# Keshav-Madhav/3d-spatial-sim-for-boid-and-nbody

Hardware: AMD Instinct MI355X
Metric: body-steps/sec (N-body Barnes-Hut, theta=0.5) (higher is better)
Workload: dtype f64 pair forces for the waves of 64 bodies whose densest quarter has G*rho*dt^2 > tau - and for every wave while most of the system qualifies (entered above a third of the waves, left below a quarter; library default 'auto') -, f32 pair forces with f64 sums for the others; f64 opening-test ties, f64; 1 GPU; galaxy_1m_bh; distribution=galaxy, bodies_per_gpu=1000000, bodies_total=1000000, method=barnes_hut, force_precision=auto, parallelism=single GPU

## Files before the change

### 3d-spatial-sim-for-boid-and-nbody_amd/csrc/common.h

```cpp
#pragma once
#include <hip/hip_runtime.h>
#include <stdint.h>
#include <stdio.h>
#include <string>

namespace nbmi {

void set_error(const char *fmt, ...);
const char *get_error();
void clear_error();

#define NBMI_HIP_CHECK(expr)                                                                \
    do {                                                                                    \
        hipError_t _e = (expr);                                                             \
        if (_e != hipSuccess) {                                                             \
            (void)hipGetLastError();  \
            nbmi::set_error("%s failed: %s (%s:%d)", #expr, hipGetErrorString(_e), __FILE__, \
                            __LINE__);                                                      \
            return -2;                                                                      \
        }                                                                                   \
    } while (0)

struct Moment {
    double m, ml, x, xl, y, yl, z, zl;
};

struct RadixConfig {
    int digit_bits = 0, threads = 0;
};
struct RadixHist;
bool radix_config_ok(RadixConfig cfg);
size_t radix_temp_bytes_u64(size_t n, int bits);
size_t radix_temp_bytes_u32(size_t n, int bits);
hipError_t radix_sort_pairs_u64(void *temp, size_t temp_bytes, const uint64_t *kin, uint64_t *kout, const uint32_t *vin,
                                uint32_t *vout, size_t n, int begin_bit, int end_bit, hipStream_t s, RadixConfig cfg = {});
hipError_t radix_sort_pairs_u32(void *temp, size_t temp_bytes, const uint32_t *kin, uint32_t *kout, const uint32_t *vin,
                                uint32_t *vout, size_t n, int begin_bit, int end_bit, hipStream_t s, RadixConfig cfg = {});
size_t radix_keys_temp_bytes_u64(size_t n, int bits);
size_t radix_keys_temp_bytes_u32(size_t n, int bits);
hipError_t radix_sort_keys_u64(void *temp, size_t temp_bytes, const uint64_t *kin, uint64_t *kout, size_t n, int begin_bit,
                               int end_bit, hipStream_t s, RadixConfig cfg = {}, bool have_hist = false);
hipError_t radix_sort_keys_u32(void *temp, size_t temp_bytes, const uint32_t *kin, uint32_t *kout, size_t n, int begin_bit,
                               int end_bit, hipStream_t s, RadixConfig cfg = {});
hipError_t radix_keys_prepare_u64(void *temp, size_t temp_bytes, size_t n, int begin_bit, int end_bit, RadixConfig cfg,
                                  hipStream_t s, RadixHist *out);
hipError_t radix_init_temp(void *temp, hipStream_t s);
hipError_t radix_error_word(const void *temp, unsigned *out, hipStream_t s);
const void *radix_error_device_word(const void *temp);

}
struct nbmi_sim;
// ... 42 lines not shown
```

### 3d-spatial-sim-for-boid-and-nbody_amd/csrc/nbmi.hip

```cpp
#include <math.h>
#include <stdarg.h>
#include <stddef.h>
#include <stdlib.h>
#include <string.h>

#include <algorithm>
#include <type_traits>
#include <utility>
#include <vector>

#include "../../include/nbmi.h"
#include "common.h"
#include "radix_hist.h"
#include "hilbert.h"
#include "visible.h"

namespace nbmi {
static thread_local char g_err[512] = "";
void set_error(const char *fmt, ...) {
    va_list ap;
    va_start(ap, fmt);
    vsnprintf(g_err, sizeof(g_err), fmt, ap);
    va_end(ap);
}
// ... 538 lines not shown
                                              double &M, double &mx, double &my, double &mz) {
    const double4 s0 = S[r], s1 = S[e];
    M = s1.x - s0.x; mx = s1.y - s0.y; my = s1.z - s0.z; mz = s1.w - s0.w;
    const int64_t ur = r >> kSubShift, ue = e >> kSubShift;
    if (ue != ur) {
        const Moment a = T[ur], b = T[ue];
        M += dd_diff(dd{b.m, b.ml}, dd{a.m, a.ml});
        mx += dd_diff(dd{b.x, b.xl}, dd{a.x, a.xl});
        my += dd_diff(dd{b.y, b.yl}, dd{a.y, a.yl});
        mz += dd_diff(dd{b.z, b.zl}, dd{a.z, a.zl});
    }
}

__device__ __forceinline__ void write_sentinel(Node *__restrict__ nodes, int32_t *__restrict__ node_ref, int64_t total,
                                               int64_t link_base = 0) {
    Node sn;
    sn.cx = sn.cy = sn.cz = 1.0e30f;
    sn.gm = 0.f; sn.s2t = 0.f;
    sn.next_off = (unsigned)(total + link_base) * kNodeBytes;
    nodes[total] = sn;
    if (node_ref) node_ref[total] = -1;
}

template <int TILE>
__global__ __launch_bounds__(kBlock) void k_emit_tile(const int32_t *__restrict__ delta, const int32_t *__restrict__ PexL,
                                                      const int32_t *__restrict__ subPex, const double4 *__restrict__ S,
                                                      const Moment *__restrict__ T, const float4 *__restrict__ posm_s,
                                                      const uint64_t *__restrict__ hi_s,
                                                      const uint64_t *__restrict__ lo_s, int64_t n, int64_t capacity,
                                                      double eps, double inv_theta2, Node *__restrict__ nodes,
                                                      Node64 *__restrict__ nodes64, uint8_t *__restrict__ node_level,
                                                      int32_t *__restrict__ node_ref, double4 *__restrict__ diag64,
                                                      NodeD *__restrict__ nodesd , Bodies cur,
                                                      const uint32_t *__restrict__ perm, double G, TreeInfo *info, int hilbert,
                                                      int64_t link_base ) {
    __shared__ uint8_t tree[2 * TILE];
    __shared__ uint8_t dprev;
    __shared__ uint32_t cells[(2 * TILE)];
    const int t = threadIdx.x;
    const int64_t base = (int64_t)blockIdx.x * TILE;
    const int64_t total = n + pex_at(PexL, subPex, n);
    if (blockIdx.x == 0 && t == 0) {
        info->num_nodes = total;
        info->walk_nodes = total;
        info->band2 = 2u * band_half_ulps(__longlong_as_double((long long)info->maxabs_bits), eps);
        if (total + 1 > capacity) {
            info->error = 1;
            if (info->sticky_error == 0) {
                info->sticky_error = 1;
                info->sticky_nodes = total;
            }
        } else {
            write_sentinel(nodes, node_ref, total, link_base);
            if (nodesd) nodesd[total] = NodeD{1.0e30, 1.0e30, 1.0e30, 0.0, 0.0f, (unsigned)(total + link_base) * kNodeDBytes};
        }
    }
    if (total + 1 > capacity) return;
    for (int i = t; i < TILE; i += kBlock) {
        const int64_t r = base + i;
        tree[TILE + i] = (uint8_t)((r < n ? delta[r] : -1) + 1);
    }
// ... 8 lines not shown
    }
    const int64_t q_tile = pex_at(PexL, subPex, base < n ? base : n);
    const int64_t tile_end = base + TILE < n ? base + TILE : n;
    const int64_t ncell = pex_at(PexL, subPex, tile_end) - q_tile;
    const int64_t nnode = (tile_end - base) + ncell;
    const int64_t idx0 = base + q_tile;
    const double bounds = info->bounds;
    const unsigned bandk = band_half_ulps(__longlong_as_double((long long)info->maxabs_bits), eps);
    for (int64_t c0 = 0; c0 < nnode; c0 += (2 * TILE)) {
        for (int i = t; i < TILE; i += kBlock) {
            const int64_t r = base + i;
            if (r >= n) break;
            const int d = (int)tree[TILE + i] - 1;
            const int dp = (int)(i > 0 ? tree[TILE + i - 1] : dprev) - 1;
            const int cnt = d > dp ? d - dp : 0;
            const int64_t s0 = i + (pex_at(PexL, subPex, r) - q_tile) - c0;
            for (int k = 0; k <= cnt; k++) {
                const int64_t c = s0 + k;
                if (c >= 0 && c < (2 * TILE)) cells[c] = ((uint32_t)i << 6) | (uint32_t)k;
            }
        }
        __syncthreads();
        const int64_t here = nnode - c0 < (2 * TILE) ? nnode - c0 : (2 * TILE);
        for (int64_t c = t; c < here; c += kBlock) {
            const uint32_t cl = cells[c];
            const int i = (int)(cl >> 6), k = (int)(cl & 63u);
            const int64_t r = base + i;
            const int64_t idx = idx0 + c0 + c;
            const int d = (int)tree[TILE + i] - 1;
            const int dp = (int)(i > 0 ? tree[TILE + i - 1] : dprev) - 1;
            const int cnt = d > dp ? d - dp : 0;
            if (k == cnt) {
                const float4 p = posm_s[r];
                Node lf;
                lf.cx = p.x; lf.cy = p.y; lf.cz = p.z; lf.gm = p.w;
                lf.s2t = 0.0f;
                lf.next_off = (unsigned)(idx + 1 + link_base) * kNodeBytes;
                nodes[idx] = lf;
                if (diag64) {
                    const uint32_t j = perm[r];
                    diag64[idx] = make_double4(cur.x[j], cur.y[j], cur.z[j], G * cur.m[j]);
                }
                if (nodesd) {
                    const uint32_t j = perm[r];
                    nodesd[idx] = NodeD{cur.x[j], cur.y[j], cur.z[j], G * cur.m[j], 0.0f, (unsigned)(idx + 1 + link_base) * kNodeDBytes};
                }
                if (node_ref) {
                    node_ref[idx] = (int32_t)r;
                    node_level[idx] = (uint8_t)((d > dp ? d : dp) + 1);
                }
                continue;
            }
            const int lev = dp + 1 + k;
            unsigned h = (unsigned)(TILE + i);
            bool found = false;
            for (;;) {
                if ((int)tree[h] <= lev) { found = true; break; }
                while ((h & 1u) && h > 1u) h >>= 1;
                if (h == 1u) break;
                h += 1u;
            }
            int64_t e;
            if (found) {
                while (h < (unsigned)TILE) {
                    h <<= 1;
                    if ((int)tree[h] > lev) h += 1u;
                }
                e = base + (int64_t)(h - (unsigned)TILE) + 1;
            } else {
                const uint64_t kh = hi_s[r];
                const bool deep = lev > 21;
                const uint64_t kl = lo_s ? lo_s[r] : (deep ? low_word_of(nullptr, cur, perm[r], hilbert, info) : 0ull);
                auto reaches = [&](int64_t u) {
                    const uint64_t hu = hi_s[u];
// ... 5 lines not shown
                    const int64_t u = ok + step;
                    if (u >= n) { bad = n; break; }
                    if (reaches(u)) { ok = u; step <<= 1; }
                    else { bad = u; break; }
                }
                while (bad - ok > 1) {
                    const int64_t mid = ok + ((bad - ok) >> 1);
                    if (reaches(mid)) ok = mid; else bad = mid;
                }
                e = bad;
            }
            double M, mx, my, mz;
            range_moments(S, T, r, e, M, mx, my, mz);
            double cx = 0.0, cy = 0.0, cz = 0.0;
            if (M > 0.0) { cx = mx / M; cy = my / M; cz = mz / M; }
            const double size = ldexp(bounds, 1 - lev);
            Node nd;
            nd.cx = (float)cx; nd.cy = (float)cy; nd.cz = (float)cz;
            nd.gm = (float)M;
            const float s2t = (float)(size * size * inv_theta2);
            nd.s2t = __int_as_float(__float_as_int(s2t) + (int)bandk);
            const int64_t nxt = e + pex_at(PexL, subPex, e) + link_base;
            nd.next_off = (unsigned)nxt * kNodeBytes;
            nodes[idx] = nd;
            if (nodesd) nodesd[idx] = NodeD{cx, cy, cz, M, __int_as_float(__float_as_int(s2t) + (int)kBand64), (unsigned)nxt * kNodeDBytes};
            nodes64[idx] = Node64{cx, cy, cz, ldexp(bounds, -lev)};
            if (diag64) diag64[idx] = make_double4(cx, cy, cz, M);
            if (node_ref) {
                node_ref[idx] = (int32_t)r;
                node_level[idx] = (uint8_t)lev;
            }
        }
        __syncthreads();
    }
}

__global__ __launch_bounds__(kBlock) void k_max_level(const int32_t *__restrict__ delta, int64_t n, TreeInfo *info) {
    __shared__ int red[kBlock / 64];
    int m = -1;
    for (int64_t i = (int64_t)blockIdx.x * kBlock + threadIdx.x; i < n; i += (int64_t)gridDim.x * kBlock) {
        const int d = delta[i];
        m = d > m ? d : m;
    }
#pragma unroll
    for (int o = 32; o > 0; o >>= 1) {
        const int other = __shfl_xor(m, o);
        m = other > m ? other : m;
    }
    if ((threadIdx.x & 63) == 0) red[threadIdx.x >> 6] = m;
    __syncthreads();
    if (threadIdx.x == 0) {
        for (int w = 1; w < kBlock / 64; w++) m = red[w] > m ? red[w] : m;
        atomicMax(&info->max_level, m + 1);
    }
// ... 2801 lines not shown
        int kind = 0;
        int64_t steps = 0, seq = 0;
    } frame_slot[NBMI_FRAME_SLOTS];
    hipStream_t frame_stream = nullptr;
    int64_t frame_seq = 0;
    uint8_t *vis_flag = nullptr;
    uint32_t *vis_slot = nullptr, *vis_tiles = nullptr;
    int xcd_chunk = 0;
    int xcd_balance = 1;
    int *xcd_bounds = nullptr;
    unsigned *wave_cycles = nullptr;
    unsigned char *wave_flag = nullptr;
    int32_t *sub_flag = nullptr;
    double step_dt = 0.0;
    double uniform_gm = -1.0;
    double max_gm = 0.0;
    int owner_all64 = -1;
    double owner_dt = 0.0;
    int balance_blocks = 0;
    hipStream_t side = nullptr;
    hipEvent_t ev_walked = nullptr, ev_cut = nullptr;
    bool cut_pending = false;
    int walk_block = kBlock;
    bool keys_lean = true;
    bool lean_build = false;
    bool sort_packed = true;
    uint64_t *packed = nullptr, *packed_s = nullptr;
    nbmi::RadixConfig sort_cfg;
    int sort_fused_hist = -1;
    int sort_bits = 0;
    bool maxabs_fused = false;
    bool fuse_maxabs = true;
    bool hilbert = true;
    double *diag_phi = nullptr;
    int32_t *diag_cnt = nullptr;
    double *diag_part = nullptr;
    long long *diag_partc = nullptr;
    double4 *diag_pot = nullptr;
    TreeInfo *side_info = nullptr;
    double *knn_r2 = nullptr, *knn_mass = nullptr;
    double4 *knn_rows = nullptr;
    unsigned long long *knn_evals = nullptr;
    int32_t *fof_parent = nullptr, *fof_root = nullptr, *fof_minid = nullptr, *fof_cnt = nullptr;
    uint32_t *fof_wleaf = nullptr;
    unsigned long long *fof_counters = nullptr;
    bool fof_ready = false, fof_cat_ready = false;
// ... 213 lines not shown
    with_bool(lean, [&](auto l) {
        k_gather_scan<decltype(l)::value><<<(int)((n_live + 1 + kScanTile - 1) / kScanTile), kBlock, 0, st>>>(
            cur, s->perm, s->hi_s, key_lo, n_live, s->G, s->posm_s, s->p64_s, lean ? nullptr : s->lo_s, s->delta, s->S, s->Pex,
            s->sub_tot, s->sub_cnt, auto_prec(s) ? s->wave_flag : nullptr, s->sub_flag,
            auto_prec(s) ? (float)(s->prec_tau / (s->step_dt * s->step_dt)) : 0.f, (float)s->softening, s->info, hil);
    });
    return 0;
}

int enqueue_global_tree(nbmi_sim *s, bool aux = true, double4 *diag = nullptr) {
    const int64_t n = s->nt;
    hipStream_t st = s->stream;
    const int64_t nsub = (n + 1 + kScanTile - 1) / kScanTile;
    k_scan_subtiles<<<1, kSubScanThreads, 0, st>>>(s->sub_tot, s->sub_cnt, nsub, s->T, s->subPex,
                                                   auto_prec(s) ? s->sub_flag : nullptr, (n + 63) / 64, s->all64_enter_pm, s->all64_leave_pm, s->info);
    const double inv_theta2 = s->theta > 0.0 ? 1.0 / (s->theta * s->theta) : INFINITY;
    const int64_t ob = s->own_base;
    const bool quad = s->multipole == NBMI_MULTIPOLE_QUADRUPOLE;
    if (quad) {
        aux = true;
        if (!diag) diag = s->quad_pot;
    }
    with_int<kEmitTileSmall, kEmitTile>(n <= kEmitSmallBodies ? kEmitTileSmall : kEmitTile, [&](auto tile) {
        constexpr int kTile = decltype(tile)::value;
        k_emit_tile<kTile><<<(int)((n + kTile - 1) / kTile), kBlock, 0, st>>>(
            s->delta, s->Pex, s->subPex, s->S, s->T, s->t_posm, s->t_hi, s->lean_build ? nullptr : s->t_lo, n,
            s->own_node_rows, s->softening, inv_theta2, s->nodes + ob, s->nodes64 + ob, aux ? s->node_level : nullptr,
            aux ? s->node_ref : nullptr, diag, s->force_prec != 1 && s->nodesd ? s->nodesd + ob : nullptr,
            s->buf[s->curbuf], s->perm, s->G, s->info, s->hilbert ? 1 : 0, ob);
    });
    if (quad && n > 0) {
        k_max_level<<<64, kBlock, 0, st>>>(s->delta, n, s->info);
        for (int lev = kMaxLevel; lev >= 0; lev--)
            k_quad_level<<<kQuadGrid, kBlock, 0, st>>>(s->nodes, s->node_level, diag, s->info, lev, s->quad_work, s->nodesq);
    }
    NBMI_HIP_CHECK(hipGetLastError());
    return 0;
}

int enqueue_tree(nbmi_sim *s, const BuildRequest &req = {}) {
    if (s->owner) {
        nbmi::set_error("this handle is in owner mode: use the nbmi_owner_* calls");
        return NBMI_ERR_ARG;
    }
    const DtScope dt_scope(s, req.step_dt);
    const bool timed = req.timing != BuildTiming::kNone;
    if (req.timing == BuildTiming::kAll) NBMI_HIP_CHECK(hipEventRecord(s->ev[0], s->stream));
    if (int rc = enqueue_maxabs(s)) return rc;
    const bool lean = s->keys_lean && req.step_dt > 0.0 && !req.aux && s->multipole != NBMI_MULTIPOLE_QUADRUPOLE;
    if (int rc = enqueue_local_sort(s, SortRequest{timed, lean})) return rc;
    if (int rc = enqueue_global_tree(s, req.aux, req.diag_rows)) return rc;
    if (timed) NBMI_HIP_CHECK(hipEventRecord(s->ev[3], s->stream));
// ... 303 lines not shown
    if (s->ev_info) (void)hipEventDestroy(s->ev_info);
    if (s->h_info) (void)hipHostFree(s->h_info);
    if (s->stream) (void)hipStreamDestroy(s->stream);
    delete s;
}

static const char *multipole_refusal(const nbmi_sim *s) {
    if (s->method != NBMI_METHOD_BARNES_HUT) return "direct N^2 handles have no cells";
    if (s->owner) return "owner-mode handles are not supported (the exchanged tree rows carry no second moments)";
    if (s->shard_begin != 0 || s->shard_end != s->n) return "sharded handles are not supported (the exchange rows carry no second moments)";
    return nullptr;
}

static void read_env_knobs(nbmi_sim *s) {
    if (const char *e = getenv("NBMI_XCD_CHUNK")) s->xcd_chunk = atoi(e);
    if (const char *e = getenv("NBMI_XCD_BALANCE")) s->xcd_balance = atoi(e);
    if (const char *e = getenv("NBMI_SPLIT_WAVES")) s->split_max_waves = atoll(e);
    if (const char *e = getenv("NBMI_WALK_PAIR")) s->walk_pair = atoi(e);
    if (const char *e = getenv("NBMI_FUSE_MAXABS")) s->fuse_maxabs = atoi(e) != 0;
    if (const char *e = getenv("NBMI_HILBERT")) s->hilbert = atoi(e) != 0;
    if (const char *e = getenv("NBMI_SORT_PACKED")) s->sort_packed = atoi(e) != 0;
    if (const char *e = getenv("NBMI_SORT_DIGIT_BITS")) s->sort_cfg.digit_bits = atoi(e);
    if (const char *e = getenv("NBMI_SORT_THREADS")) s->sort_cfg.threads = atoi(e);
    if (const char *e = getenv("NBMI_SORT_FUSED_HIST")) s->sort_fused_hist = atoi(e) != 0 ? 1 : 0;
    if (const char *e = getenv("NBMI_KEYS_LEAN")) s->keys_lean = atoi(e) != 0;
    if (const char *e = getenv("NBMI_PAIRS_CELLS")) s->pair_cells = atoi(e) != 0;
    if (const char *e = getenv("NBMI_FORCE_PREC")) {
        const int v = atoi(e);
        if (v >= 0 && v <= 2) s->force_prec = v;
    }
    if (const char *e = getenv("NBMI_PREC_TAU")) s->prec_tau = atof(e);
    if (const char *e = getenv("NBMI_MULTIPOLE")) {
        if (!strcmp(e, "quadrupole") || !strcmp(e, "1")) s->multipole_env = NBMI_MULTIPOLE_QUADRUPOLE;
    }
    if (const char *e = getenv("NBMI_ALL64_ENTER")) s->all64_enter_pm = (int)(1000.0 * atof(e) + 0.5);
    if (const char *e = getenv("NBMI_ALL64_LEAVE")) s->all64_leave_pm = (int)(1000.0 * atof(e) + 0.5);
    if (const char *e = getenv("NBMI_SORT_BITS")) {
        const int b = atoi(e);
        if (b >= 8 && b <= 63) s->sort_bits = b;
    }
    if (const char *e = getenv("NBMI_WALK_BLOCK")) {
        const int b = atoi(e);
        if (b == 64 || b == 128 || b == 256) s->walk_block = b;
    }
}

static nbmi_sim *create_failed(nbmi_sim *s) {
    std::string keep = nbmi::get_error();
    nbmi_destroy(s);
    nbmi::set_error("%s", keep.c_str());
    return nullptr;
}

static int create_impl(nbmi_sim *s, const double *pos, const double *vel, const double *mass) {
    const int64_t n = s->n;
    const int64_t c = s->cap > n ? s->cap : n;
    if (!nbmi::radix_config_ok(s->sort_cfg)) {
        nbmi::set_error("NBMI_SORT_DIGIT_BITS must be 8 or 10 and NBMI_SORT_THREADS 256, 512 or 1024 (got %d, %d)", s->sort_cfg.digit_bits,
                        s->sort_cfg.threads);
        return NBMI_ERR_ARG;
    }
    NBMI_HIP_CHECK(hipSetDevice(s->device));
    NBMI_HIP_CHECK(hipStreamCreateWithFlags(&s->stream, hipStreamNonBlocking));
    for (auto &e : s->ev) NBMI_HIP_CHECK(hipEventCreate(&e));
    if (alloc_bodies(s, &s->buf[0], c) || alloc_bodies(s, &s->buf[1], c)) return -2;
    if (dev_alloc(s, &s->posm_s, c) || dev_alloc(s, &s->colors, 3 * (c ? c : 1)) || dev_alloc(s, &s->info, 1)) return -2;
    void *stage = nullptr;
    NBMI_HIP_CHECK(hipMalloc(&stage, (size_t)(c ? c : 1) * 7 * sizeof(double)));
    s->allocs.push_back(stage);
    s->stage = stage;
    NBMI_HIP_CHECK(hipMemsetAsync(s->info, 0, sizeof(TreeInfo), s->stream));
    NBMI_HIP_CHECK(hipMemsetAsync(s->colors, 0, (size_t)(c ? c : 1) * 3 * sizeof(float), s->stream));
    if (s->method == NBMI_METHOD_BARNES_HUT) {
        s->node_capacity = node_rows_for(c) + s->node_extra;
        const int64_t own_rows = node_rows_for(c);
        if (dev_alloc(s, &s->key_hi, c) || dev_alloc(s, &s->key_lo, c) || dev_alloc(s, &s->hi_s, c) ||
            dev_alloc(s, &s->lo_s, c) ||
            (s->sort_packed && !s->owner && (dev_alloc(s, &s->packed, c) || dev_alloc(s, &s->packed_s, c))) || (s->owner && dev_alloc(s, &s->p64_s, c)) || dev_alloc(s, &s->idx, c) ||
            dev_alloc(s, &s->perm, c) || dev_alloc(s, &s->delta, c) || dev_alloc(s, &s->Pex, c + 1) ||
            dev_alloc(s, &s->S, c + 1) || dev_alloc(s, &s->sub_tot, (c + 1) / kScanTile + 2) ||
            dev_alloc(s, &s->sub_cnt, (c + 1) / kScanTile + 2) || dev_alloc(s, &s->subPex, (c + 1) / kScanTile + 2) ||
            dev_alloc(s, &s->T, (c + 1) / kScanTile + 2) ||
// ... 1698 lines not shown
```

### 3d-spatial-sim-for-boid-and-nbody_amd/csrc/radix.hip

```cpp
#include <hip/hip_runtime.h>
#include <stdint.h>

#include <type_traits>

#include "common.h"
#include "radix_hist.h"
#include "scan.h"
#include <stddef.h>

namespace nbmi {
namespace {

constexpr int kItems = 16, kItemsMin = 4;
constexpr int kWideTile = 4096;
constexpr unsigned kFlagAgg = 1u << 30, kFlagIncl = 2u << 30, kValueMask = (1u << 30) - 1;
#ifndef NBMI_LOOK_BATCH
#define NBMI_LOOK_BATCH 8
#endif
constexpr int kLookBatch = NBMI_LOOK_BATCH;
constexpr int kMaxPasses = kRadixMaxPasses;
constexpr size_t kLargeMinKeys = 524288, kWideMaxKeys = 2097152;
constexpr int kLargeThreads = 512, kWideThreads = 1024;

struct Control {
    unsigned error;
    unsigned pad0[15];
    unsigned tile_ticket[kMaxPasses];
    unsigned pad[8];
    unsigned hist[kMaxPasses * kRadixMaxBins];
};

template <typename K>
__device__ __forceinline__ unsigned digit_of(K k, int shift, unsigned dmask) {
    return (unsigned)(k >> shift) & dmask;
}

constexpr int kHistThreads = 256;
template <typename K>
__global__ __launch_bounds__(kHistThreads) void k_radix_hist(const K *__restrict__ keys, int64_t n, int bits, int first_bit,
                                                            int digit_bits, Control *ctl) {
    const int passes = radix_passes(bits, digit_bits);
    extern __shared__ unsigned h[];
    for (int i = threadIdx.x; i < (passes << digit_bits); i += kHistThreads) h[i] = 0u;
    __syncthreads();
    for (int64_t i = (int64_t)blockIdx.x * kHistThreads + threadIdx.x; i < n; i += (int64_t)gridDim.x * kHistThreads)
        radix_hist_count(h, (uint64_t)(keys[i] >> first_bit), bits, digit_bits, passes);
    __syncthreads();
    radix_hist_flush(h, ctl->hist, digit_bits, passes, kHistThreads);
}

template <int OWN>
__device__ __forceinline__ void status_load(const unsigned *p, unsigned (&w)[OWN]) {
    if constexpr (OWN == 1) {
        w[0] = __hip_atomic_load(p, __ATOMIC_RELAXED, __HIP_MEMORY_SCOPE_AGENT);
    } else {
#pragma unroll
        for (int o = 0; o < OWN; o += 2) {
            const unsigned long long v = __hip_atomic_load(reinterpret_cast<const unsigned long long *>(p + o), __ATOMIC_RELAXED,
                                                           __HIP_MEMORY_SCOPE_AGENT);
            w[o] = (unsigned)v;
            w[o + 1] = (unsigned)(v >> 32);
        }
    }
}
template <int OWN>
__device__ __forceinline__ void status_store(unsigned *p, unsigned flag, const unsigned (&v)[OWN]) {
    if constexpr (OWN == 1) {
        __hip_atomic_store(p, flag | v[0], __ATOMIC_RELAXED, __HIP_MEMORY_SCOPE_AGENT);
    } else {
#pragma unroll
        for (int o = 0; o < OWN; o += 2)
            __hip_atomic_store(reinterpret_cast<unsigned long long *>(p + o),
                               (unsigned long long)(flag | v[o]) | ((unsigned long long)(flag | v[o + 1]) << 32), __ATOMIC_RELAXED,
                               __HIP_MEMORY_SCOPE_AGENT);
    }
}

template <typename K, int BITS, int THREADS, int ITEMS, bool kPairs, int LOOK = kLookBatch>
__global__ __launch_bounds__(THREADS) void k_radix_pass(const K *__restrict__ kin, K *__restrict__ kout,
                                                       const uint32_t *__restrict__ vin, uint32_t *__restrict__ vout,
                                                       int64_t n, int shift, unsigned dmask, int pass, Control *ctl,
                                                       unsigned *__restrict__ status ) {
    constexpr int BINS = 1 << BITS, WAVES = THREADS / 64, TILE = THREADS * ITEMS;
    constexpr int OWN = BINS > THREADS ? BINS / THREADS : 1;
    static_assert(TILE <= 65536 && (OWN == 1 || OWN % 2 == 0), "16-bit slots; owned status words go in 8-byte accesses");
    using cnt_t = typename std::conditional<(BITS > 8), uint16_t, unsigned>::type;
    __shared__ unsigned s_tile;
    __shared__ cnt_t cnt_w[WAVES][BINS];
    __shared__ unsigned tile_off[BINS];
    __shared__ unsigned glob_off[BINS];
    __shared__ K lds_k[TILE];

    const int t = threadIdx.x, lane = t & 63, w = t >> 6;
    const bool owner = BINS >= THREADS || t < BINS;
    const int d0 = t * OWN;
    if (t == 0) s_tile = atomicAdd(&ctl->tile_ticket[pass], 1u);
    for (int i = t; i < (int)(sizeof(cnt_w) / sizeof(unsigned)); i += THREADS) reinterpret_cast<unsigned *>(&cnt_w[0][0])[i] = 0u;
    unsigned graw[OWN];
#pragma unroll
    for (int o = 0; o < OWN; o++) graw[o] = owner ? ctl->hist[(pass << BITS) + d0 + o] : 0u;
    __syncthreads();
    const unsigned tile = s_tile;
    const int64_t tile_base = (int64_t)tile * TILE;
    const int valid_in_tile = (int)((n - tile_base) < TILE ? (n - tile_base) : TILE);

// ... 44 lines not shown
        tsum += run;
        gsum += graw[o];
    }
    const unsigned long long ex =
        scan::block_scan<THREADS>(((unsigned long long)tsum << 32) | gsum, 0ull, scan::Sum()).excl;
    unsigned my_tile_off[OWN], my_glob[OWN];
    {
        unsigned rt = (unsigned)(ex >> 32), rg = (unsigned)ex;
#pragma unroll
        for (int o = 0; o < OWN; o++) {
            my_tile_off[o] = rt;
            my_glob[o] = rg;
            rt += total[o];
            rg += graw[o];
            if (owner) tile_off[d0 + o] = my_tile_off[o];
        }
    }

    unsigned prefix[OWN];
#pragma unroll
    for (int o = 0; o < OWN; o++) prefix[o] = 0u;
    if (owner) {
        unsigned *mine = status + (size_t)tile * BINS + d0;
        if (tile == 0) {
            status_store<OWN>(mine, kFlagIncl, total);
        } else {
            status_store<OWN>(mine, kFlagAgg, total);
            constexpr unsigned kAll = (1u << OWN) - 1u;
            int p = (int)tile - 1;
            unsigned spins = 0;
            unsigned done = 0;
            while (done != kAll) {
                unsigned sw[LOOK][OWN];
#pragma unroll
                for (int j = 0; j < LOOK; j++) {
                    const int q = p - j;
                    if (q >= 0) {
                        status_load<OWN>(status + (size_t)q * BINS + d0, sw[j]);
                    } else {
#pragma unroll
                        for (int o = 0; o < OWN; o++) sw[j][o] = kFlagIncl;
                    }
                }
#pragma unroll
                for (int j = 0; j < LOOK; j++) {
                    if (done == kAll) break;
                    bool ready = true;
#pragma unroll
                    for (int o = 0; o < OWN; o++)
                        if (!((done >> o) & 1u) && (sw[j][o] & ~kValueMask) == 0u) ready = false;
                    if (!ready) {
                        if (++spins > (1u << 22)) { ctl->error = 1u; done = kAll; }
                        __builtin_amdgcn_s_sleep(2);
                        break;
                    }
#pragma unroll
                    for (int o = 0; o < OWN; o++) {
                        if ((done >> o) & 1u) continue;
                        prefix[o] += sw[j][o] & kValueMask;
                        if ((sw[j][o] & ~kValueMask) == kFlagIncl) done |= 1u << o;
                    }
                    p--;
                }
            }
            unsigned incl[OWN];
#pragma unroll
            for (int o = 0; o < OWN; o++) incl[o] = prefix[o] + total[o];
            status_store<OWN>(mine, kFlagIncl, incl);
        }
#pragma unroll
        for (int o = 0; o < OWN; o++) glob_off[d0 + o] = my_glob[o] + prefix[o] - my_tile_off[o];
    }
    __syncthreads();

    unsigned slot[kPairs ? (ITEMS + 1) / 2 : 1];
#pragma unroll
    for (int i = 0; i < ITEMS; i++) {
        const int64_t idx = wave_base + i * 64 + lane;
        unsigned q = 0;
        if (idx < n) {
            const unsigned d = digit_of(key[i], shift, dmask);
            q = tile_off[d] + (unsigned)cnt_w[w][d] + rank[i];
            lds_k[q] = key[i];
        }
        if (kPairs) {
            if (i & 1) slot[i >> 1] |= q << 16; else slot[i >> 1] = q;
        }
    }
    __syncthreads();
    unsigned dst[kPairs ? ITEMS : 1];
#pragma unroll
// ... 5 lines not shown
            kout[g] = k;
            if (kPairs) dst[i] = g;
        }
    }
    if (!kPairs) return;
    __syncthreads();
    uint32_t *lds_v = reinterpret_cast<uint32_t *>(lds_k);
#pragma unroll
    for (int i = 0; i < ITEMS; i++) {
        const int64_t idx = wave_base + i * 64 + lane;
        if (idx < n) lds_v[(slot[i >> 1] >> ((i & 1) * 16)) & 0xffffu] = val[i];
    }
    __syncthreads();
#pragma unroll
    for (int i = 0; i < ITEMS; i++) {
        const int q = i * THREADS + t;
        if (q < valid_in_tile) vout[dst[i]] = lds_v[q];
    }
}

inline size_t tiles_for(size_t n, size_t tile) { return (n + tile - 1) / tile; }
inline size_t align256(size_t b) { return (b + 255) & ~(size_t)255; }

inline size_t status_bytes_max(size_t n, int bits) {
    const size_t narrow = (size_t)radix_passes(bits, 8) * tiles_for(n, 256 * kItemsMin) * 256;
    const size_t wide = (size_t)radix_passes(bits, kRadixMaxBits) * tiles_for(n, kWideTile) * kRadixMaxBins;
    return align256((narrow > wide ? narrow : wide) * sizeof(unsigned));
}

template <typename K, bool kPairs = true>
size_t temp_bytes(size_t n, int bits) {
    return align256(sizeof(Control)) + status_bytes_max(n, bits) + align256(n * sizeof(K)) +
           (kPairs ? align256(n * sizeof(uint32_t)) : 0);
}

struct Shape {
    int bits = 0, threads = 0, items = 0;
    size_t tile() const { return (size_t)threads * items; }
};
inline bool resolve_shape(RadixConfig want, size_t n, int field_bits, bool pairs, Shape *out) {
    if ((want.digit_bits != 0 && want.digit_bits != 8 && want.digit_bits != 10) ||
        (want.threads != 0 && want.threads != 256 && want.threads != 512 && want.threads != 1024))
        return false;
    Shape s;
    const bool large = !pairs && n > kLargeMinKeys;
    const bool wide = large && n <= kWideMaxKeys && !want.digit_bits && !want.threads &&
                      (field_bits % 10 == 0 || radix_passes(field_bits, 10) < radix_passes(field_bits, 8));
    s.bits = want.digit_bits ? want.digit_bits : (wide ? 10 : 8);
    s.threads = want.threads ? want.threads : (wide ? kWideThreads : (large ? kLargeThreads : 256));
    if (s.bits == 8 && s.threads == 256) s.items = n <= 65536 ? kItemsMin : (n <= 524288 ? 8 : kItems);
    else s.items = kWideTile / s.threads;
    *out = s;
    return true;
}

template <typename K, bool kPairs>
hipError_t check_sort(size_t temp_size, size_t n, int bits, RadixConfig want, Shape *shape) {
    if (n > (size_t)kValueMask) return hipErrorInvalidValue;
    if (bits < 1 || !resolve_shape(want, n, bits, kPairs, shape)) return hipErrorInvalidValue;
    const int passes = radix_passes(bits, shape->bits);
    if (passes < 1 || passes > kMaxPasses || temp_size < temp_bytes<K, kPairs>(n, bits)) return hipErrorInvalidValue;
    return hipSuccess;
}

inline hipError_t clear_sort(char *base, size_t n, int bits, const Shape &shape, hipStream_t st) {
    const size_t rows = (size_t)radix_passes(bits, shape.bits) * tiles_for(n, shape.tile());
    return hipMemsetAsync(base + offsetof(Control, tile_ticket), 0,
                          align256(sizeof(Control)) - offsetof(Control, tile_ticket) + rows * ((size_t)sizeof(unsigned) << shape.bits), st);
}

template <typename K, int BITS, int THREADS, int ITEMS, bool kPairs>
void launch_pass(size_t tiles, hipStream_t st, const K *ksrc, K *kdst, const uint32_t *vsrc, uint32_t *vdst, int64_t n, int shift,
                 unsigned dmask, int p, Control *ctl, unsigned *status) {
    k_radix_pass<K, BITS, THREADS, ITEMS, kPairs><<<(int)tiles, THREADS, 0, st>>>(ksrc, kdst, vsrc, vdst, n, shift, dmask, p, ctl, status);
}

template <typename K, bool kPairs>
hipError_t sort_impl(void *temp, size_t temp_size, const K *kin, K *kout, const uint32_t *vin, uint32_t *vout,
                     size_t n, int begin_bit, int end_bit, RadixConfig want, bool have_hist, hipStream_t st) {
    const int bits = end_bit - begin_bit;
    if (n == 0) return hipSuccess;
    Shape shape;
    if (hipError_t e = check_sort<K, kPairs>(temp_size, n, bits, want, &shape)) return e;
    const int passes = radix_passes(bits, shape.bits);
    char *base = (char *)temp;
    Control *ctl = (Control *)base;
    const size_t tiles = tiles_for(n, shape.tile());
    unsigned *status = (unsigned *)(base + align256(sizeof(Control)));
    K *ktmp = (K *)((char *)status + status_bytes_max(n, bits));
    uint32_t *vtmp = kPairs ? (uint32_t *)((char *)ktmp + align256(n * sizeof(K))) : nullptr;
    if (!have_hist) {
        if (hipError_t e = clear_sort(base, n, bits, shape, st)) return e;
        int hb = (int)((n + kHistThreads * 8 - 1) / (kHistThreads * 8));
        if (hb > 1024) hb = 1024;
        k_radix_hist<K><<<hb, kHistThreads, ((size_t)passes << shape.bits) * sizeof(unsigned), st>>>(kin, (int64_t)n, bits, begin_bit,
                                                                                                    shape.bits, ctl);
    }
    const K *ksrc = kin;
    const uint32_t *vsrc = vin;
    for (int p = 0; p < passes; p++) {
        const bool to_out = ((passes - 1 - p) % 2) == 0;
        K *kdst = to_out ? kout : ktmp;
        uint32_t *vdst = to_out ? vout : vtmp;
        const int shift = begin_bit + p * shape.bits;
        const unsigned dmask = radix_digit_mask(bits, shape.bits, p);
        unsigned *srow = status + ((size_t)p * tiles << shape.bits);
#define NBMI_PASS(B, T, I)                                                                                                 \
    if (shape.bits == B && shape.threads == T && shape.items == I)                                                        \
        launch_pass<K, B, T, I, kPairs>(tiles, st, ksrc, kdst, vsrc, vdst, (int64_t)n, shift, dmask, p, ctl, srow)
        NBMI_PASS(8, 256, 4);
        NBMI_PASS(8, 256, 8);
        NBMI_PASS(8, 256, 16);
        NBMI_PASS(8, 512, 8);
        NBMI_PASS(8, 1024, 4);
        NBMI_PASS(10, 256, 16);
        NBMI_PASS(10, 512, 8);
        NBMI_PASS(10, 1024, 4);
#undef NBMI_PASS
        ksrc = kdst;
        vsrc = vdst;
    }
    return hipGetLastError();
}

template <typename K>
hipError_t sort_keys(void *temp, size_t temp_size, const K *kin, K *kout, size_t n, int begin_bit, int end_bit,
                     RadixConfig want, bool have_hist, hipStream_t st) {
    if (begin_bit < 0 || end_bit > (int)(8 * sizeof(K)) || begin_bit >= end_bit) return hipErrorInvalidValue;
    return sort_impl<K, false>(temp, temp_size, kin, kout, nullptr, nullptr, n, begin_bit, end_bit, want, have_hist, st);
}

}
// ... 45 lines not shown
```

### 3d-spatial-sim-for-boid-and-nbody_amd/csrc/sortscan.hip

```cpp
#include <cstdlib>
#include <cstring>

#include "../../include/nbmi.h"
#include "common.h"

static void *g_tmp = nullptr;
static size_t g_tmp_bytes = 0;
static hipError_t debug_temp(size_t need, hipStream_t st, void **out) {
    if (need > g_tmp_bytes) {
        if (g_tmp) (void)hipFree(g_tmp);
        g_tmp = nullptr;
        g_tmp_bytes = 0;
        if (hipError_t e = hipMalloc(&g_tmp, need)) return e;
        g_tmp_bytes = need;
        if (hipError_t e = nbmi::radix_init_temp(g_tmp, st)) return e;
    }
    *out = g_tmp;
    return hipSuccess;
}

static int debug_sort(const char *who, int key_bytes, int64_t n, const void *keys, const uint32_t *values, void *keys_out,
                      uint32_t *values_out, int begin_bit, int end_bit, int repeats, double *ms_per_sort,
                      nbmi::RadixConfig cfg = {}) {
    if (n == 0) return 0;
// ... 59 lines not shown

extern "C" int nbmi_debug_sort_pairs(int key_bytes, int64_t n, const void *keys, const uint32_t *values, void *keys_out,
                                     uint32_t *values_out, int bits, int impl, int repeats, double *ms_per_sort) {
    if ((key_bytes != 4 && key_bytes != 8) || n < 0 || bits < 1 || bits > 8 * key_bytes || (n && (!keys || !values)) || impl != 0) {
        nbmi::set_error("nbmi_debug_sort_pairs: bad arguments");
        return NBMI_ERR_ARG;
    }
    return debug_sort("nbmi_debug_sort_pairs", key_bytes, n, keys, values, keys_out, values_out, 0, bits, repeats, ms_per_sort);
}

extern "C" int nbmi_debug_sort_keys(int key_bytes, int64_t n, const void *keys, void *keys_out, int begin_bit, int end_bit,
                                    int repeats, double *ms_per_sort) {
    if ((key_bytes != 4 && key_bytes != 8) || n < 0 || begin_bit < 0 || end_bit <= begin_bit || end_bit > 8 * key_bytes ||
        end_bit - begin_bit > 64 || (n && (!keys || !keys_out))) {
        nbmi::set_error("nbmi_debug_sort_keys: bad arguments");
        return NBMI_ERR_ARG;
    }
    return debug_sort("nbmi_debug_sort_keys", key_bytes, n, keys, nullptr, keys_out, nullptr, begin_bit, end_bit, repeats, ms_per_sort);
}

extern "C" int nbmi_debug_sort_config(int key_bytes, int64_t n, const void *keys, const uint32_t *values, void *keys_out,
                                      uint32_t *values_out, int begin_bit, int end_bit, int digit_bits, int threads, int repeats,
                                      double *ms_per_sort) {
    const nbmi::RadixConfig cfg{digit_bits, threads};
    if ((key_bytes != 4 && key_bytes != 8) || n < 0 || begin_bit < 0 || end_bit <= begin_bit || end_bit > 8 * key_bytes ||
        (n && (!keys || !keys_out)) || (n && values && !values_out) || !nbmi::radix_config_ok(cfg)) {
        nbmi::set_error("nbmi_debug_sort_config: bad arguments");
        return NBMI_ERR_ARG;
    }
    return debug_sort("nbmi_debug_sort_config", key_bytes, n, keys, values, keys_out, values_out, begin_bit, end_bit, repeats, ms_per_sort,
                      cfg);
}
```

Measured before the change: 515.6 million body-steps/s.

## Stage emitted tree nodes in LDS and add two-level radix look-back

The tree-emit kernel can now stage each batch of Node/NodeD records in shared memory and write them out as aligned 16-byte coalesced stretches, on by default. It also gets occupancy hints through waves_per_eu, replacing scattered per-thread struct stores with wide contiguous ones at the cost of extra LDS and barriers. Separately, the radix sort's decoupled look-back gains a group-level status row, so a tile can skip back over 16 tiles at a time once a group aggregate is published. Grouping is automatic for mid-sized tile counts, and it needs extra status memory and more complex flag logic.

```diff
diff --git a/3d-spatial-sim-for-boid-and-nbody_amd/csrc/common.h b/3d-spatial-sim-for-boid-and-nbody_amd/csrc/common.h
--- a/3d-spatial-sim-for-boid-and-nbody_amd/csrc/common.h
+++ b/3d-spatial-sim-for-boid-and-nbody_amd/csrc/common.h
@@ -26,7 +26,7 @@
 };
 
 struct RadixConfig {
-    int digit_bits = 0, threads = 0;
+    int digit_bits = 0, threads = 0, look_group = 0;
 };
 struct RadixHist;
 bool radix_config_ok(RadixConfig cfg);
diff --git a/3d-spatial-sim-for-boid-and-nbody_amd/csrc/nbmi.hip b/3d-spatial-sim-for-boid-and-nbody_amd/csrc/nbmi.hip
--- a/3d-spatial-sim-for-boid-and-nbody_amd/csrc/nbmi.hip
+++ b/3d-spatial-sim-for-boid-and-nbody_amd/csrc/nbmi.hip
@@ -584,8 +584,21 @@
     if (node_ref) node_ref[total] = -1;
 }
 
-template <int TILE>
-__global__ __launch_bounds__(kBlock) void k_emit_tile(const int32_t *__restrict__ delta, const int32_t *__restrict__ PexL,
+__device__ __forceinline__ void store_stretch(unsigned long long *__restrict__ dst, const unsigned long long *src, int units, int t) {
+    const int head = (int)((reinterpret_cast<uintptr_t>(dst) >> 3) & 1u);
+    if (units <= 0) return;
+    if (head && t == 0) dst[0] = src[0];
+    const int pairs = (units - head) >> 1;
+    for (int u = t; u < pairs; u += kBlock) {
+        const int a = head + 2 * u;
+        *reinterpret_cast<ulonglong2 *>(dst + a) = make_ulonglong2(src[a], src[a + 1]);
+    }
+    const int tail = head + 2 * pairs;
+    if (tail < units && t == kBlock - 1) dst[tail] = src[tail];
+}
+
+template <int TILE, bool kStaged>
+__global__ __launch_bounds__(kBlock) __attribute__((amdgpu_waves_per_eu(TILE > kEmitTileSmall ? 6 : 5, 8))) void k_emit_tile(const int32_t *__restrict__ delta, const int32_t *__restrict__ PexL,
                                                       const int32_t *__restrict__ subPex, const double4 *__restrict__ S,
                                                       const Moment *__restrict__ T, const float4 *__restrict__ posm_s,
                                                       const uint64_t *__restrict__ hi_s,
@@ -599,6 +612,9 @@
     __shared__ uint8_t tree[2 * TILE];
     __shared__ uint8_t dprev;
     __shared__ uint32_t cells[(2 * TILE)];
+    constexpr int kNodeUnits = kNodeBytes / 8, kNodeDUnits = kNodeDBytes / 8;
+    __shared__ unsigned long long stage_n[kStaged ? kBlock * kNodeUnits : 1];
+    __shared__ unsigned long long stage_d[kStaged ? kBlock * kNodeDUnits : 1];
     const int t = threadIdx.x;
     const int64_t base = (int64_t)blockIdx.x * TILE;
     const int64_t total = n + pex_at(PexL, subPex, n);
@@ -653,7 +669,13 @@
         }
         __syncthreads();
         const int64_t here = nnode - c0 < (2 * TILE) ? nnode - c0 : (2 * TILE);
-        for (int64_t c = t; c < here; c += kBlock) {
+        auto put_node = [&](int64_t idx, const Node &v) {
+            if constexpr (kStaged) reinterpret_cast<Node *>(stage_n)[t] = v; else nodes[idx] = v;
+        };
+        auto put_noded = [&](int64_t idx, const NodeD &v) {
+            if constexpr (kStaged) reinterpret_cast<NodeD *>(stage_d)[t] = v; else nodesd[idx] = v;
+        };
+        auto emit_node = [&](int64_t c) {
             const uint32_t cl = cells[c];
             const int i = (int)(cl >> 6), k = (int)(cl & 63u);
             const int64_t r = base + i;
@@ -667,20 +689,20 @@
                 lf.cx = p.x; lf.cy = p.y; lf.cz = p.z; lf.gm = p.w;
                 lf.s2t = 0.0f;
                 lf.next_off = (unsigned)(idx + 1 + link_base) * kNodeBytes;
-                nodes[idx] = lf;
+                put_node(idx, lf);
                 if (diag64) {
                     const uint32_t j = perm[r];
                     diag64[idx] = make_double4(cur.x[j], cur.y[j], cur.z[j], G * cur.m[j]);
                 }
                 if (nodesd) {
                     const uint32_t j = perm[r];
-                    nodesd[idx] = NodeD{cur.x[j], cur.y[j], cur.z[j], G * cur.m[j], 0.0f, (unsigned)(idx + 1 + link_base) * kNodeDBytes};
+                    put_noded(idx, NodeD{cur.x[j], cur.y[j], cur.z[j], G * cur.m[j], 0.0f, (unsigned)(idx + 1 + link_base) * kNodeDBytes});
                 }
                 if (node_ref) {
                     node_ref[idx] = (int32_t)r;
                     node_level[idx] = (uint8_t)((d > dp ? d : dp) + 1);
                 }
-                continue;
+                return;
             }
             const int lev = dp + 1 + k;
             unsigned h = (unsigned)(TILE + i);
@@ -732,14 +754,27 @@
             nd.s2t = __int_as_float(__float_as_int(s2t) + (int)bandk);
             const int64_t nxt = e + pex_at(PexL, subPex, e) + link_base;
             nd.next_off = (unsigned)nxt * kNodeBytes;
-            nodes[idx] = nd;
-            if (nodesd) nodesd[idx] = NodeD{cx, cy, cz, M, __int_as_float(__float_as_int(s2t) + (int)kBand64), (unsigned)nxt * kNodeDBytes};
+            put_node(idx, nd);
+            if (nodesd) put_noded(idx, NodeD{cx, cy, cz, M, __int_as_float(__float_as_int(s2t) + (int)kBand64), (unsigned)nxt * kNodeDBytes});
             nodes64[idx] = Node64{cx, cy, cz, ldexp(bounds, -lev)};
             if (diag64) diag64[idx] = make_double4(cx, cy, cz, M);
             if (node_ref) {
                 node_ref[idx] = (int32_t)r;
                 node_level[idx] = (uint8_t)lev;
             }
+        };
+        if constexpr (kStaged) {
+            for (int64_t cb = 0; cb < here; cb += kBlock) {
+                if (cb + t < here) emit_node(cb + t);
+                __syncthreads();
+                const int cnt = (int)(here - cb < kBlock ? here - cb : kBlock);
+                const int64_t first = idx0 + c0 + cb;
+                store_stretch(reinterpret_cast<unsigned long long *>(nodes + first), stage_n, cnt * kNodeUnits, t);
+                if (nodesd) store_stretch(reinterpret_cast<unsigned long long *>(nodesd + first), stage_d, cnt * kNodeDUnits, t);
+                __syncthreads();
+            }
+        } else {
+            for (int64_t c = t; c < here; c += kBlock) emit_node(c);
         }
         __syncthreads();
     }
@@ -3587,6 +3622,7 @@
     hipEvent_t ev_walked = nullptr, ev_cut = nullptr;
     bool cut_pending = false;
     int walk_block = kBlock;
+    bool emit_staged = true;
     bool keys_lean = true;
     bool lean_build = false;
     bool sort_packed = true;
@@ -3846,12 +3882,14 @@
         if (!diag) diag = s->quad_pot;
     }
     with_int<kEmitTileSmall, kEmitTile>(n <= kEmitSmallBodies ? kEmitTileSmall : kEmitTile, [&](auto tile) {
-        constexpr int kTile = decltype(tile)::value;
-        k_emit_tile<kTile><<<(int)((n + kTile - 1) / kTile), kBlock, 0, st>>>(
-            s->delta, s->Pex, s->subPex, s->S, s->T, s->t_posm, s->t_hi, s->lean_build ? nullptr : s->t_lo, n,
-            s->own_node_rows, s->softening, inv_theta2, s->nodes + ob, s->nodes64 + ob, aux ? s->node_level : nullptr,
-            aux ? s->node_ref : nullptr, diag, s->force_prec != 1 && s->nodesd ? s->nodesd + ob : nullptr,
-            s->buf[s->curbuf], s->perm, s->G, s->info, s->hilbert ? 1 : 0, ob);
+        with_bool(s->emit_staged, [&](auto staged) {
+            constexpr int kTile = decltype(tile)::value;
+            k_emit_tile<kTile, decltype(staged)::value><<<(int)((n + kTile - 1) / kTile), kBlock, 0, st>>>(
+                s->delta, s->Pex, s->subPex, s->S, s->T, s->t_posm, s->t_hi, s->lean_build ? nullptr : s->t_lo, n,
+                s->own_node_rows, s->softening, inv_theta2, s->nodes + ob, s->nodes64 + ob, aux ? s->node_level : nullptr,
+                aux ? s->node_ref : nullptr, diag, s->force_prec != 1 && s->nodesd ? s->nodesd + ob : nullptr,
+                s->buf[s->curbuf], s->perm, s->G, s->info, s->hilbert ? 1 : 0, ob);
+        });
     });
     if (quad && n > 0) {
         k_max_level<<<64, kBlock, 0, st>>>(s->delta, n, s->info);
@@ -4201,8 +4239,10 @@
     if (const char *e = getenv("NBMI_SORT_PACKED")) s->sort_packed = atoi(e) != 0;
     if (const char *e = getenv("NBMI_SORT_DIGIT_BITS")) s->sort_cfg.digit_bits = atoi(e);
     if (const char *e = getenv("NBMI_SORT_THREADS")) s->sort_cfg.threads = atoi(e);
+    if (const char *e = getenv("NBMI_SORT_LOOK_GROUP")) s->sort_cfg.look_group = atoi(e);
     if (const char *e = getenv("NBMI_SORT_FUSED_HIST")) s->sort_fused_hist = atoi(e) != 0 ? 1 : 0;
     if (const char *e = getenv("NBMI_KEYS_LEAN")) s->keys_lean = atoi(e) != 0;
+    if (const char *e = getenv("NBMI_EMIT_STAGED")) s->emit_staged = atoi(e) != 0;
     if (const char *e = getenv("NBMI_PAIRS_CELLS")) s->pair_cells = atoi(e) != 0;
     if (const char *e = getenv("NBMI_FORCE_PREC")) {
         const int v = atoi(e);
@@ -4235,8 +4275,8 @@
     const int64_t n = s->n;
     const int64_t c = s->cap > n ? s->cap : n;
     if (!nbmi::radix_config_ok(s->sort_cfg)) {
-        nbmi::set_error("NBMI_SORT_DIGIT_BITS must be 8 or 10 and NBMI_SORT_THREADS 256, 512 or 1024 (got %d, %d)", s->sort_cfg.digit_bits,
-                        s->sort_cfg.threads);
+        nbmi::set_error("NBMI_SORT_DIGIT_BITS must be 8 or 10, NBMI_SORT_THREADS 256, 512 or 1024 and NBMI_SORT_LOOK_GROUP 0, 1 or 16 "
+                        "(got %d, %d, %d)", s->sort_cfg.digit_bits, s->sort_cfg.threads, s->sort_cfg.look_group);
         return NBMI_ERR_ARG;
     }
     NBMI_HIP_CHECK(hipSetDevice(s->device));
diff --git a/3d-spatial-sim-for-boid-and-nbody_amd/csrc/radix.hip b/3d-spatial-sim-for-boid-and-nbody_amd/csrc/radix.hip
--- a/3d-spatial-sim-for-boid-and-nbody_amd/csrc/radix.hip
+++ b/3d-spatial-sim-for-boid-and-nbody_amd/csrc/radix.hip
@@ -18,6 +18,12 @@
 #define NBMI_LOOK_BATCH 8
 #endif
 constexpr int kLookBatch = NBMI_LOOK_BATCH;
+#ifndef NBMI_LOOK_GROUP
+#define NBMI_LOOK_GROUP 16
+#endif
+constexpr int kLookGroup = NBMI_LOOK_GROUP;
+static_assert(kLookGroup > 1 && kLookGroup % kLookBatch == 0 && (kLookGroup & (kLookGroup - 1)) == 0,
+              "a group is a whole number of look-back batches (and a power of two: tile -> group is a shift)");
 constexpr int kMaxPasses = kRadixMaxPasses;
 constexpr size_t kLargeMinKeys = 524288, kWideMaxKeys = 2097152;
 constexpr int kLargeThreads = 512, kWideThreads = 1024;
@@ -64,23 +70,27 @@
     }
 }
 template <int OWN>
-__device__ __forceinline__ void status_store(unsigned *p, unsigned flag, const unsigned (&v)[OWN]) {
+__device__ __forceinline__ void status_store(unsigned *p, unsigned flag, const unsigned (&v)[OWN], unsigned done_mask = 0u,
+                                             unsigned flag_done = 0u) {
+    unsigned w[OWN];
+#pragma unroll
+    for (int o = 0; o < OWN; o++) w[o] = (((done_mask >> o) & 1u) ? flag_done : flag) | v[o];
     if constexpr (OWN == 1) {
-        __hip_atomic_store(p, flag | v[0], __ATOMIC_RELAXED, __HIP_MEMORY_SCOPE_AGENT);
+        __hip_atomic_store(p, w[0], __ATOMIC_RELAXED, __HIP_MEMORY_SCOPE_AGENT);
     } else {
 #pragma unroll
         for (int o = 0; o < OWN; o += 2)
-            __hip_atomic_store(reinterpret_cast<unsigned long long *>(p + o),
-                               (unsigned long long)(flag | v[o]) | ((unsigned long long)(flag | v[o + 1]) << 32), __ATOMIC_RELAXED,
-                               __HIP_MEMORY_SCOPE_AGENT);
-    }
-}
-
-template <typename K, int BITS, int THREADS, int ITEMS, bool kPairs, int LOOK = kLookBatch>
+            __hip_atomic_store(reinterpret_cast<unsigned long long *>(p + o), (unsigned long long)w[o] | ((unsigned long long)w[o + 1] << 32),
+                               __ATOMIC_RELAXED, __HIP_MEMORY_SCOPE_AGENT);
+    }
+}
+
+template <typename K, int BITS, int THREADS, int ITEMS, bool kPairs, bool kTwo, int LOOK = kLookBatch>
 __global__ __launch_bounds__(THREADS) void k_radix_pass(const K *__restrict__ kin, K *__restrict__ kout,
                                                        const uint32_t *__restrict__ vin, uint32_t *__restrict__ vout,
                                                        int64_t n, int shift, unsigned dmask, int pass, Control *ctl,
-                                                       unsigned *__restrict__ status ) {
+                                                       unsigned *__restrict__ status ,
+                                                       unsigned *__restrict__ gstatus ) {
     constexpr int BINS = 1 << BITS, WAVES = THREADS / 64, TILE = THREADS * ITEMS;
     constexpr int OWN = BINS > THREADS ? BINS / THREADS : 1;
     static_assert(TILE <= 65536 && (OWN == 1 || OWN % 2 == 0), "16-bit slots; owned status words go in 8-byte accesses");
@@ -171,21 +181,43 @@
     for (int o = 0; o < OWN; o++) prefix[o] = 0u;
     if (owner) {
         unsigned *mine = status + (size_t)tile * BINS + d0;
+        constexpr int G = kTwo ? kLookGroup : 1;
+        const bool glast = kTwo && (tile % G) == G - 1;
+        unsigned *gmine = kTwo ? gstatus + (size_t)(tile / G) * BINS + d0 : nullptr;
         if (tile == 0) {
             status_store<OWN>(mine, kFlagIncl, total);
         } else {
             status_store<OWN>(mine, kFlagAgg, total);
             constexpr unsigned kAll = (1u << OWN) - 1u;
             int p = (int)tile - 1;
+            bool gpub = false;
             unsigned spins = 0;
             unsigned done = 0;
-            while (done != kAll) {
+            while (done != kAll && p >= 0) {
+                const unsigned *rows = status;
+                int q0 = p, left = LOOK, step = 1;
+                if constexpr (kTwo) {
+                    left = (p + 1) % G;
+                    if (left == 0) {
+                        if (glast && !gpub) {
+                            gpub = true;
+                            unsigned gsum[OWN];
+#pragma unroll
+                            for (int o = 0; o < OWN; o++) gsum[o] = prefix[o] + total[o];
+                            status_store<OWN>(gmine, kFlagAgg, gsum, done, kFlagIncl);
+                        }
+                        rows = gstatus;
+                        q0 = (p + 1) / G - 1;
+                        left = LOOK;
+                        step = G;
+                    }
+                }
                 unsigned sw[LOOK][OWN];
 #pragma unroll
                 for (int j = 0; j < LOOK; j++) {
-                    const int q = p - j;
-                    if (q >= 0) {
-                        status_load<OWN>(status + (size_t)q * BINS + d0, sw[j]);
+                    const int q = q0 - j;
+                    if (j < left && q >= 0) {
+                        status_load<OWN>(rows + (size_t)q * BINS + d0, sw[j]);
                     } else {
 #pragma unroll
                         for (int o = 0; o < OWN; o++) sw[j][o] = kFlagIncl;
@@ -193,7 +225,7 @@
                 }
 #pragma unroll
                 for (int j = 0; j < LOOK; j++) {
-                    if (done == kAll) break;
+                    if (done == kAll || j >= left) break;
                     bool ready = true;
 #pragma unroll
                     for (int o = 0; o < OWN; o++)
@@ -209,13 +241,14 @@
                         prefix[o] += sw[j][o] & kValueMask;
                         if ((sw[j][o] & ~kValueMask) == kFlagIncl) done |= 1u << o;
                     }
-                    p--;
+                    p -= step;
                 }
             }
             unsigned incl[OWN];
 #pragma unroll
             for (int o = 0; o < OWN; o++) incl[o] = prefix[o] + total[o];
             status_store<OWN>(mine, kFlagIncl, incl);
+            if (glast) status_store<OWN>(gmine, kFlagIncl, incl);
         }
 #pragma unroll
         for (int o = 0; o < OWN; o++) glob_off[d0 + o] = my_glob[o] + prefix[o] - my_tile_off[o];
@@ -267,9 +300,11 @@
 inline size_t tiles_for(size_t n, size_t tile) { return (n + tile - 1) / tile; }
 inline size_t align256(size_t b) { return (b + 255) & ~(size_t)255; }
 
+inline size_t group_rows(size_t tiles, int group) { return group > 1 ? tiles / (size_t)group : 0; }
 inline size_t status_bytes_max(size_t n, int bits) {
-    const size_t narrow = (size_t)radix_passes(bits, 8) * tiles_for(n, 256 * kItemsMin) * 256;
-    const size_t wide = (size_t)radix_passes(bits, kRadixMaxBits) * tiles_for(n, kWideTile) * kRadixMaxBins;
+    const size_t tn = tiles_for(n, 256 * kItemsMin), tw = tiles_for(n, kWideTile);
+    const size_t narrow = (size_t)radix_passes(bits, 8) * (tn + group_rows(tn, kLookGroup)) * 256;
+    const size_t wide = (size_t)radix_passes(bits, kRadixMaxBits) * (tw + group_rows(tw, kLookGroup)) * kRadixMaxBins;
     return align256((narrow > wide ? narrow : wide) * sizeof(unsigned));
 }
 
@@ -281,11 +316,14 @@
 
 struct Shape {
     int bits = 0, threads = 0, items = 0;
+    int group = 1;
     size_t tile() const { return (size_t)threads * items; }
 };
+constexpr size_t kTwoMinTiles = 4 * kLookGroup, kTwoMaxTiles = 512;
 inline bool resolve_shape(RadixConfig want, size_t n, int field_bits, bool pairs, Shape *out) {
     if ((want.digit_bits != 0 && want.digit_bits != 8 && want.digit_bits != 10) ||
-        (want.threads != 0 && want.threads != 256 && want.threads != 512 && want.threads != 1024))
+        (want.threads != 0 && want.threads != 256 && want.threads != 512 && want.threads != 1024) ||
+        (want.look_group != 0 && want.look_group != 1 && want.look_group != kLookGroup))
         return false;
     Shape s;
     const bool large = !pairs && n > kLargeMinKeys;
@@ -295,6 +333,8 @@
     s.threads = want.threads ? want.threads : (wide ? kWideThreads : (large ? kLargeThreads : 256));
     if (s.bits == 8 && s.threads == 256) s.items = n <= 65536 ? kItemsMin : (n <= 524288 ? 8 : kItems);
     else s.items = kWideTile / s.threads;
+    const size_t tiles = tiles_for(n, s.tile());
+    s.group = want.look_group ? want.look_group : (tiles >= kTwoMinTiles && tiles <= kTwoMaxTiles ? kLookGroup : 1);
     *out = s;
     return true;
 }
@@ -309,15 +349,21 @@
 }
 
 inline hipError_t clear_sort(char *base, size_t n, int bits, const Shape &shape, hipStream_t st) {
-    const size_t rows = (size_t)radix_passes(bits, shape.bits) * tiles_for(n, shape.tile());
+    const size_t tiles = tiles_for(n, shape.tile());
+    const size_t rows = (size_t)radix_passes(bits, shape.bits) * (tiles + group_rows(tiles, shape.group));
     return hipMemsetAsync(base + offsetof(Control, tile_ticket), 0,
                           align256(sizeof(Control)) - offsetof(Control, tile_ticket) + rows * ((size_t)sizeof(unsigned) << shape.bits), st);
 }
 
 template <typename K, int BITS, int THREADS, int ITEMS, bool kPairs>
 void launch_pass(size_t tiles, hipStream_t st, const K *ksrc, K *kdst, const uint32_t *vsrc, uint32_t *vdst, int64_t n, int shift,
-                 unsigned dmask, int p, Control *ctl, unsigned *status) {
-    k_radix_pass<K, BITS, THREADS, ITEMS, kPairs><<<(int)tiles, THREADS, 0, st>>>(ksrc, kdst, vsrc, vdst, n, shift, dmask, p, ctl, status);
+                 unsigned dmask, int p, Control *ctl, unsigned *status, unsigned *gstatus ) {
+    if (gstatus)
+        k_radix_pass<K, BITS, THREADS, ITEMS, kPairs, true><<<(int)tiles, THREADS, 0, st>>>(ksrc, kdst, vsrc, vdst, n, shift, dmask, p, ctl,
+                                                                                          status, gstatus);
+    else
+        k_radix_pass<K, BITS, THREADS, ITEMS, kPairs, false><<<(int)tiles, THREADS, 0, st>>>(ksrc, kdst, vsrc, vdst, n, shift, dmask, p, ctl,
+                                                                                           status, nullptr);
 }
 
 template <typename K, bool kPairs>
@@ -350,9 +396,10 @@
         const int shift = begin_bit + p * shape.bits;
         const unsigned dmask = radix_digit_mask(bits, shape.bits, p);
         unsigned *srow = status + ((size_t)p * tiles << shape.bits);
+        unsigned *grow = shape.group > 1 ? status + (((size_t)passes * tiles + (size_t)p * group_rows(tiles, shape.group)) << shape.bits) : nullptr;
 #define NBMI_PASS(B, T, I)                                                                                                 \
     if (shape.bits == B && shape.threads == T && shape.items == I)                                                        \
-        launch_pass<K, B, T, I, kPairs>(tiles, st, ksrc, kdst, vsrc, vdst, (int64_t)n, shift, dmask, p, ctl, srow)
+        launch_pass<K, B, T, I, kPairs>(tiles, st, ksrc, kdst, vsrc, vdst, (int64_t)n, shift, dmask, p, ctl, srow, grow)
         NBMI_PASS(8, 256, 4);
         NBMI_PASS(8, 256, 8);
         NBMI_PASS(8, 256, 16);
diff --git a/3d-spatial-sim-for-boid-and-nbody_amd/csrc/sortscan.hip b/3d-spatial-sim-for-boid-and-nbody_amd/csrc/sortscan.hip
--- a/3d-spatial-sim-for-boid-and-nbody_amd/csrc/sortscan.hip
+++ b/3d-spatial-sim-for-boid-and-nbody_amd/csrc/sortscan.hip
@@ -105,7 +105,8 @@
 extern "C" int nbmi_debug_sort_config(int key_bytes, int64_t n, const void *keys, const uint32_t *values, void *keys_out,
                                       uint32_t *values_out, int begin_bit, int end_bit, int digit_bits, int threads, int repeats,
                                       double *ms_per_sort) {
-    const nbmi::RadixConfig cfg{digit_bits, threads};
+    nbmi::RadixConfig cfg{digit_bits, threads};
+    if (const char *e = getenv("NBMI_SORT_LOOK_GROUP")) cfg.look_group = atoi(e);
     if ((key_bytes != 4 && key_bytes != 8) || n < 0 || begin_bit < 0 || end_bit <= begin_bit || end_bit > 8 * key_bytes ||
         (n && (!keys || !keys_out)) || (n && values && !values_out) || !nbmi::radix_config_ok(cfg)) {
         nbmi::set_error("nbmi_debug_sort_config: bad arguments");
```

Result: no change. 518.5 million body-steps/s (median of 6 runs) (+0.6%).
